# lizaibeim/mmla-audio

Measured on AMD Instinct MI355X. Metric: audio clips/sec (MFCC→logits) at 1/2/4/8 MI355X; MFCC max-abs-err vs librosa, higher is better.
Workload: dtype f16x3+f32

## Files before the change

### mmla_audio_amd/csrc/context.cpp

```cpp
#include <algorithm>
#include <cstdarg>
#include <cstdio>
#include <cstdlib>

#include "internal.h"

using namespace mmla;

namespace mmla __attribute__((visibility("hidden"))) {

int fail(mmla_ctx* c, int code, const char* fmt, ...) {
  char buf[512];
  va_list ap;
  va_start(ap, fmt);
  vsnprintf(buf, sizeof(buf), fmt, ap);
  va_end(ap);
  if (c) c->err = buf;
  return code;
}

static hipEvent_t prof_event(mmla_ctx* c) {
  if (!c->prof_pool.empty()) {
    hipEvent_t e = c->prof_pool.back();
    c->prof_pool.pop_back();
// ... 75 lines not shown
  }
  *out = c->ws[slot];
  return MMLA_OK;
}

int ws_release(mmla_ctx* c) {
  HIPCHK(c, hipStreamSynchronize(c->stream));
  for (size_t i = 0; i < c->ws.size(); ++i)
    if (c->ws[i]) {
      HIPCHK(c, hipFree(static_cast<char*>(c->ws[i]) - c->ws_guard[i]));
      c->ws[i] = nullptr;
      c->ws_size[i] = 0;
      c->ws_guard[i] = 0;
    }
  return MMLA_OK;
}

static int ws_check_guards(mmla_ctx* c) {
  std::vector<unsigned char> h(kGuardBytes);
  for (size_t slot = 0; slot < c->ws.size(); ++slot) {
    const size_t g = c->ws_guard[slot];
    if (!c->ws[slot] || !g) continue;
    for (int side = 0; side < 2; ++side) {
      const char* d = static_cast<const char*>(c->ws[slot]) + (side ? c->ws_size[slot] : -(ptrdiff_t)g);
      HIPCHK(c, hipMemcpy(h.data(), d, g, hipMemcpyDeviceToHost));
      for (size_t i = 0; i < g; ++i)
        if (h[i] != kGuardByte)
          return fail(c, MMLA_E_HIP, "workspace slot %zu: %s guard overwritten at byte %zu", slot,
                      side ? "trailing" : "leading", side ? i : g - i);
    }
  }
  return MMLA_OK;
}

int finish(mmla_ctx* c, bool dev) {
  HIPCHK(c, hipGetLastError());
  bool guarded = false;
  for (size_t g : c->ws_guard) guarded |= g != 0;
  if (!dev || guarded) HIPCHK(c, hipStreamSynchronize(c->stream));
  if (guarded) return ws_check_guards(c);
  return MMLA_OK;
}

constexpr double kOdBytesPerClip = 3.0 * 128 * 151 * 32 * 4 + 128 * 151 * 3 + 128 * 151 * 4 +
                                   19 * 128 * 4 + 512 * 4 + 64;
constexpr double kSiBytesPerClip = 4.0 * 256 * 32 * 4 + 256 * 39 * 4 + 8 * 128 * 4 + 512 * 4 +
                                   1024 * 4 + 64;

int64_t microbatch(mmla_ctx* c, bool od) {
  const int64_t user = od ? c->od_mb : c->si_mb;
  if (user > 0) return user;
  const int64_t cap = od ? c->od_mb_cap : c->si_mb_cap;
  size_t fr = 0, tot = 0;
  if (hipMemGetInfo(&fr, &tot) != hipSuccess) {
    (void)hipGetLastError();
    return cap;
  }
  double held = 0;
  for (size_t b : c->ws_size) held += (double)b;
  int64_t fit = (int64_t)(((double)fr + held) * 0.9 / (od ? kOdBytesPerClip : kSiBytesPerClip));
  fit = fit / kMinMicrobatch * kMinMicrobatch;
  return std::max(kMinMicrobatch, std::min(cap, fit));
}

}

struct EnvSwitch {
  const char* name;
  bool mmla_ctx::*no;
  int mmla_ctx::*num;
};
static const EnvSwitch kEnvSwitches[] = {
    {"MMLA_DEBUG_FAIL_ALLOC", nullptr, &mmla_ctx::debug_fail_allocs},
    {"MMLA_NO_SIU", &mmla_ctx::siu, nullptr},
    {"MMLA_NO_SIPU", &mmla_ctx::sipu, nullptr},
    {"MMLA_NO_SIFIN", &mmla_ctx::sifin, nullptr},
    {"MMLA_NO_SIPAIR", &mmla_ctx::sipair, nullptr},
    {"MMLA_NO_SICHAIN", &mmla_ctx::sichain, nullptr},
    {"MMLA_NO_LSTM_SPLIT", &mmla_ctx::lstm_split, nullptr},
    {"MMLA_LSTM_SPLIT_MAX", nullptr, &mmla_ctx::lstm_split_max},
    {"MMLA_DEBUG_LSTM_SPIN", nullptr, &mmla_ctx::lstm_spin},
    {"MMLA_NO_SIPAD", &mmla_ctx::si_pad_feat, nullptr},
    {"MMLA_NO_ODU", &mmla_ctx::odu, nullptr},
    {"MMLA_RB_TILE", &mmla_ctx::rbs, nullptr},
    {"MMLA_NO_PIN_OUT", &mmla_ctx::pin_small, nullptr},
};

extern "C" {

int mmla_abi_version(void) { return MMLA_ABI_VERSION; }

int mmla_create(int device, mmla_ctx** out) {
  if (!out) return MMLA_E_INVALID;
  *out = nullptr;
  int ndev = 0;
  if (hipGetDeviceCount(&ndev) != hipSuccess || ndev == 0) return MMLA_E_HIP;
  if (device < 0 || device >= ndev) return MMLA_E_INVALID;
  if (hipSetDevice(device) != hipSuccess) return MMLA_E_HIP;
  mmla_ctx* c = new mmla_ctx();
  c->device = device;
  for (const EnvSwitch& s : kEnvSwitches)
    if (const char* v = std::getenv(s.name)) {
      if (s.no) c->*s.no = std::atoi(v) == 0;
      else c->*s.num = std::atoi(v);
    }
  if (hipStreamCreateWithFlags(&c->own_stream, hipStreamDefault) != hipSuccess) {
    delete c;
    return MMLA_E_HIP;
  }
  c->stream = c->own_stream;
  if (hipMalloc(&c->range_dev, 4 * sizeof(int)) != hipSuccess ||
      hipMemset(c->range_dev, 0, 4 * sizeof(int)) != hipSuccess ||
      hipHostMalloc(&c->range_host, 2 * sizeof(int), hipHostMallocDefault) != hipSuccess) {
    mmla_destroy(c);
    return MMLA_E_HIP;
  }
  if (c->pin_small) {
    const unsigned fl = hipHostMallocMapped | hipHostMallocCoherent;
    if (hipHostMalloc(reinterpret_cast<void**>(&c->range_map), 64, fl) != hipSuccess ||
        hipHostGetDevicePointer(reinterpret_cast<void**>(&c->range_map_dev), c->range_map, 0) != hipSuccess ||
        hipHostMalloc(reinterpret_cast<void**>(&c->pin_out), kPinSlots * kPinSlotBytes, fl) != hipSuccess ||
        hipHostGetDevicePointer(reinterpret_cast<void**>(&c->pin_out_dev), c->pin_out, 0) != hipSuccess ||
        hipHostMalloc(reinterpret_cast<void**>(&c->pin_in), kPinInBytes, hipHostMallocDefault) != hipSuccess) {
      mmla_destroy(c);
      return MMLA_E_HIP;
    }
    c->range_map[0] = c->range_map[1] = 0;
  }
  OdFeTables ot;
  od_fe_build_tables(&ot);
  if (!od_fe_tables_ok(ot)) {
    mmla_destroy(c);
    return MMLA_E_INVALID;
  }
  SiFeTables st;
  si_fe_build_tables(&st);
  if (!si_fe_tables_ok(st)) {
    mmla_destroy(c);
    return MMLA_E_INVALID;
  }
  if (hipMalloc(&c->od_tables, sizeof(OdFeTables)) != hipSuccess ||
      hipMalloc(&c->si_tables, sizeof(SiFeTables)) != hipSuccess ||
      hipMemcpy(c->od_tables, &ot, sizeof(ot), hipMemcpyHostToDevice) != hipSuccess ||
      hipMemcpy(c->si_tables, &st, sizeof(st), hipMemcpyHostToDevice) != hipSuccess) {
    mmla_destroy(c);
    return MMLA_E_HIP;
  }
  *out = c;
  return MMLA_OK;
}

int mmla_destroy(mmla_ctx* c) {
  if (!c) return MMLA_E_INVALID;
  (void)hipSetDevice(c->device);
  if (c->stream) (void)hipStreamSynchronize(c->stream);
  free_allocs(c->od_allocs);
  free_allocs(c->si_allocs);
  for (size_t i = 0; i < c->ws.size(); ++i)
    if (c->ws[i]) (void)hipFree(static_cast<char*>(c->ws[i]) - c->ws_guard[i]);
  if (c->od_tables) (void)hipFree(c->od_tables);
  if (c->si_tables) (void)hipFree(c->si_tables);
  if (c->nr_tables) (void)hipFree(c->nr_tables);
  if (c->nr_thresh) (void)hipFree(c->nr_thresh);
  if (c->range_dev) (void)hipFree(c->range_dev);
  if (c->vad_state) (void)hipFree(c->vad_state);
  if (c->range_host) (void)hipHostFree(c->range_host);
// ... 121 lines not shown
```

### mmla_audio_amd/csrc/internal.h

```cpp
#pragma once
#include <hip/hip_runtime.h>

#include <cstdint>
#include <cstring>
#include <string>
#include <vector>

#include "../../include/mmla.h"
#include "nr.h"
#include "od_fe.h"
#include "si_fe.h"
#include "vad.h"

namespace mmla __attribute__((visibility("hidden"))) {

constexpr int OD_H = 128, OD_W = 151, OD_PIX = OD_H * OD_W;
constexpr int OD_IMG = OD_PIX * 3;
constexpr int SI_T = 256, SI_D = 39;
constexpr int SI_NEED_SAMPLES = 160 * 259 + 400;
constexpr int CH[9] = {32, 32, 32, 64, 64, 64, 128, 128, 128};
constexpr bool POOL[9] = {true, false, false, true, false, false, true, false, false};

struct ConvW {
  float* wt = nullptr;
// ... 5 lines not shown
  int kh = 0, kw = 0, cin = 0, cout = 0, cout_pad = 0, cin_pad = 0, kpad = 0;
  float wscale = 256.0f;
  float unscale() const { return 1.0f / (16.0f * wscale); }
};
struct BnW {
  float* scale = nullptr;
  float* shift = nullptr;
  int c = 0;
};
struct LstmW {
  float* wcat[2] = {nullptr, nullptr};
  float* bias[2] = {nullptr, nullptr};
  uint16_t* wth[2] = {nullptr, nullptr};
  uint16_t* wtl[2] = {nullptr, nullptr};
  float ws[2] = {256.0f, 256.0f};
};
struct ResUnitW {
  BnW bn_in, bn_mid;
  ConvW ca, cb, sc;
};
struct OdNet {
  ConvW stem;
  ResUnitW blk[9];
  LstmW lstm;
  float* head_w = nullptr;
  float* head_b = nullptr;
};
struct SiNet {
  ConvW stem;
  ResUnitW unit[9];
  BnW final_bn;
  LstmW lstm;
  ConvW dense;
  int k = 0, head = 0;
};

struct ProfRec {
  int stage;
  hipEvent_t a, b;
  double work;
};

constexpr int64_t kOdMicrobatch = 16384;
constexpr int64_t kSiMicrobatch = 65536;
constexpr int64_t kMinMicrobatch = 64;

constexpr size_t kPinSlotBytes = 64u << 10;
constexpr size_t kPinInBytes = 1u << 20;
constexpr int kPinSlots = 4;

}

struct mmla_ctx {
  bool prof_on = false;
  std::vector<mmla::ProfRec> prof_pending;
  std::vector<hipEvent_t> prof_pool;
  double prof_ms[MMLA_NSTAGES] = {0};
  double prof_work[MMLA_NSTAGES] = {0};
  int64_t prof_n[MMLA_NSTAGES] = {0};
  int device = 0;
  hipStream_t stream = nullptr;
  hipStream_t own_stream = nullptr;
  std::string err;
  OdFeTables* od_tables = nullptr;
  SiFeTables* si_tables = nullptr;
  bool od_loaded = false, si_loaded = false;
  mmla::OdNet od;
  mmla::SiNet si;
  std::vector<void*> od_allocs, si_allocs;
  std::vector<void*> ws;
  std::vector<size_t> ws_size;
  std::vector<size_t> ws_guard;
  int64_t od_mb = 0, si_mb = 0;
  int64_t od_mb_cap = mmla::kOdMicrobatch, si_mb_cap = mmla::kSiMicrobatch;
  int debug_fail_allocs = 0;
  int precision = MMLA_PREC_F16X3;
  bool siu = true;
  bool sipu = true;
  bool sifin = true;
  bool sipair = true;
  bool sichain = true;
  bool si_pad_feat = true;
  bool odu = true;
  bool rbs = true;
  bool lstm_split = true;
  int lstm_split_max = 128;
  int lstm_spin = 0;
  int* range_dev = nullptr;
  int* range_host = nullptr;
  bool pin_small = true;
  int* range_map = nullptr;
  int* range_map_dev = nullptr;
  char* pin_out = nullptr;
  char* pin_out_dev = nullptr;
  char* pin_in = nullptr;
  int* range_ptr = nullptr;
  int* timeout_ptr = nullptr;
  int64_t lstm_split_reruns = 0;
  int64_t range_reruns = 0;
  bool od_f32_only = false, si_f32_only = false;
  bool loading_f16_bad = false;
  VadState* vad_state = nullptr;
  int64_t vad_streams = 0;
  NrTables* nr_tables = nullptr;
  float* nr_thresh = nullptr;
  bool nr_ready = false;
};

namespace mmla __attribute__((visibility("hidden"))) {

int fail(mmla_ctx* c, int code, const char* fmt, ...);

#define HIPCHK(ctx, expr)                                                                        \
  do {                                                                                           \
    hipError_t e_ = (expr);                                                                      \
    if (e_ != hipSuccess)                                                                        \
      return mmla::fail(ctx, MMLA_E_HIP, "%s failed: %s (%s:%d)", #expr, hipGetErrorString(e_), \
                        __FILE__, __LINE__);                                                     \
  } while (0)

#define CHK(expr)              \
  do {                         \
    int r_ = (expr);           \
    if (r_ != MMLA_OK) return r_; \
  } while (0)

int prof_begin(mmla_ctx* c, int stage);
void prof_end(mmla_ctx* c, int idx, double work);
int prof_collect(mmla_ctx* c);

#define LAUNCH(c, st, wk, expr)                  \
  do {                                           \
    const int pi_ = mmla::prof_begin((c), (st)); \
    HIPCHK((c), (expr));                         \
    mmla::prof_end((c), pi_, (wk));              \
  } while (0)

enum Slot {
  S_PCM = 0, S_LENS, S_IMG, S_X, S_T1, S_T2, S_T3, S_SEQ, S_HOUT, S_LOGIT, S_FEAT, S_SILENT,
  S_OUT0, S_OUT1, S_OUT2, S_OUT3, S_IN,
  S_NR_S, S_NR_BITS, S_NR_FMAX, S_NR_FRAMES, S_NR_ITEMS, S_NR_Y, S_NR_ROWS,
  S_VAD_SPEECH, S_VAD_OUT, S_VAD_LENS, S_RS_TR, S_RS_WIN, S_LSTM,
  S_TRAIN
};

int ws_get(mmla_ctx* c, int slot, size_t bytes, void** out);
int ws_release(mmla_ctx* c);
int64_t microbatch(mmla_ctx* c, bool od);
int finish(mmla_ctx* c, bool dev);
void free_allocs(std::vector<void*>& al);

template <typename T>
int in_ptr(mmla_ctx* c, const T* user, size_t count, bool dev, int slot, const T** d) {
  *d = user;
  if (dev || !user) return MMLA_OK;
  void* p = nullptr;
  CHK(ws_get(c, slot, count * sizeof(T), &p));
  HIPCHK(c, hipMemcpyAsync(p, user, count * sizeof(T), hipMemcpyHostToDevice, c->stream));
  *d = static_cast<const T*>(p);
  return MMLA_OK;
}

template <typename T>
int out_ptr(mmla_ctx* c, T* user, int64_t off, size_t count, bool dev, int slot, T** d) {
  if (!user) {
    *d = nullptr;
// ... 45 lines not shown
```

### mmla_audio_amd/csrc/net_runners.cpp

```cpp
#include <algorithm>

#include "conv.h"
#include "conv_h3.h"
#include "internal.h"
#include "nets.h"
#include "odu.h"
#include "resblk.h"
#include "siu.h"

using namespace mmla;

namespace {

ConvArgs conv_args(const ConvW& w, const float* x, float* y, int n, int h, int wd, int stride,
                   const BnW* bn, int pro, int epi, const float* res) {
  ConvArgs a{};
  a.x = x;
  a.wt = w.wt;
  a.bias = w.bias;
  a.scale = bn ? bn->scale : nullptr;
  a.shift = bn ? bn->shift : nullptr;
  a.res = res;
  a.y = y;
  a.n = n;
  a.h = h;
  a.w = wd;
  a.cin = w.cin;
  a.ho = (h + stride - 1) / stride;
  a.wo = (wd + stride - 1) / stride;
  a.cout = w.cout;
  a.cout_pad = w.cout_pad;
  a.ldy = w.cout;
  a.kh = w.kh;
  a.kw = w.kw;
  a.stride = stride;
  const int th = std::max((a.ho - 1) * stride + w.kh - h, 0);
  const int tw = std::max((a.wo - 1) * stride + w.kw - wd, 0);
  a.pad_h = th / 2;
  a.pad_w = tw / 2;
  a.pro = pro;
  a.epi = epi;
  return a;
}

double conv_flops(const ConvArgs& a) {
  return 2.0 * (double)a.n * a.ho * a.wo * a.kh * a.kw * a.cin * a.cout;
}

int conv_run(mmla_ctx* c, const ConvArgs& a, int stage = MMLA_STAGE_CONV) {
  LAUNCH(c, stage, conv_flops(a), conv_launch(a, c->stream));
  return MMLA_OK;
}

ConvH3Args conv_h3_args(const ConvW& w, const float* x, float* y, int n, int h, int wd, const BnW* bn,
                        int pro, int epi, const float* res, int* range_flag) {
  ConvH3Args a{};
  a.x = x;
  a.wh = w.wh;
  a.wl = w.wl;
  a.unscale = w.unscale();
  a.bias = w.bias;
  a.scale = bn ? bn->scale : nullptr;
  a.shift = bn ? bn->shift : nullptr;
  a.res = res;
  a.y = y;
  a.n = n;
  a.h = h;
  a.w = wd;
  a.cin = w.cin;
  a.cin_pad = w.cin_pad;
  a.cout = w.cout;
  a.cout_pad = w.cout_pad;
  a.kh = w.kh;
  a.kw = w.kw;
  a.pad_h = (w.kh - 1) / 2;
  a.pad_w = (w.kw - 1) / 2;
  a.pro = pro;
  a.epi = epi;
  a.range_flag = range_flag;
  return a;
}

int conv_spatial(mmla_ctx* c, const ConvW& w, const float* x, float* y, int n, int h, int wd,
                 const BnW* bn, int pro, int epi, const float* res, bool pool_out = false,
                 int pool_in_h = 0, const ConvW* sc = nullptr, const float* sc_x = nullptr,
                 int sc_h = 0) {
  if (c->precision == MMLA_PREC_F16X3 && w.wh) {
    ConvH3Args a = conv_h3_args(w, x, y, n, h, wd, bn, pro, epi, res, c->range_ptr);
    double sc_flops = 0.0;
    if (sc && sc_x) {
      a.sc_x = sc_x;
      a.sc_wh = sc->wh;
      a.sc_wl = sc->wl;
      a.sc_bias = sc->bias;
      a.sc_cin = sc->cin;
      a.sc_h = sc_h;
      a.sc_unscale = sc->unscale();
      sc_flops = sc_h > 0 ? 2.0 * n * h * sc->cin * sc->cout
                          : 2.0 * n * ((h + 1) / 2) * ((wd + 1) / 2) * sc->cin * sc->cout;
    }
    a.pool_in = pool_in_h > 0;
    a.h_in = pool_in_h;
    a.pool_out = pool_out ? 1 : 0;
    LAUNCH(c, MMLA_STAGE_CONV, 2.0 * n * h * wd * w.kh * w.kw * w.cin * w.cout + sc_flops,
           conv_h3_launch(a, c->stream));
    return MMLA_OK;
  }
  ConvArgs a = conv_args(w, x, y, n, h, wd, 1, bn, pro, epi, res);
  if (!pool_out) return conv_run(c, a);
  return fail(c, MMLA_E_INVALID, "pooled epilogue needs the 3xFP16 conv path");
}

int ws_floats(mmla_ctx* c, int slot, size_t count, float** out) {
  void* p = nullptr;
  CHK(ws_get(c, slot, count * sizeof(float), &p));
  *out = static_cast<float*>(p);
  return MMLA_OK;
}

double lstm_flops(int64_t n, int T, int D) { return 2.0 * n * T * 2 * (256.0 + D) * 1024.0; }

hipError_t lstm_run(mmla_ctx* c, const LstmW& L, const float* seq, int64_t n, int T, float* out) {
  if (c->precision == MMLA_PREC_F16X3 && L.wth[0] && c->lstm_split &&
      n <= std::min(c->lstm_split_max, bilstm_h3_split_max_clips())) {
    void* ws = nullptr;
    if (ws_get(c, S_LSTM, bilstm_h3_split_ws_bytes(), &ws) != MMLA_OK) return hipErrorOutOfMemory;
    return bilstm_h3_split_launch(seq, (int)n, T, 128, L.wth[0], L.wtl[0], L.wth[1], L.wtl[1],
                                  L.bias[0], L.bias[1], out, c->range_ptr, L.ws[0], L.ws[1], ws,
                                  c->timeout_ptr, c->lstm_spin, c->stream);
  }
  if (c->precision == MMLA_PREC_F16X3 && L.wth[0])
    return bilstm_h3_launch(seq, (int)n, T, 128, L.wth[0], L.wtl[0], L.wth[1], L.wtl[1], L.bias[0],
                            L.bias[1], out, c->range_ptr, L.ws[0], L.ws[1], c->stream);
  return bilstm_launch(seq, (int)n, T, 128, L.wcat[0], L.wcat[1], L.bias[0], L.bias[1], out,
                       c->stream);
}


enum OdPath {
  OD_STRIPS,
  OD_TILES,
  OD_ODU,
  OD_PAIR
};
struct OdChoice {
  OdPath path;
  bool stem;
};

bool strips_ok(const ResUnitW& B, bool pool, int h, int w) {
  return B.ca.wh && B.cb.wh && (!pool || B.sc.wh) && B.ca.cin_pad == B.ca.cin && B.ca.cout_pad == 32 &&
         B.cb.cin_pad == 32 && B.cb.cout_pad == 32 && B.cb.kh == 4 && B.cb.kw == 1 &&
         (!pool || (B.sc.cin_pad == B.ca.cin && B.sc.cout_pad == 32)) &&
         rbs_supported(h, w, B.ca.cin, B.ca.cout, pool);
}

bool tiles_ok(const ResUnitW& B, bool pool) {
  return B.ca.fh && B.cb.fh && B.cb.kpad == 4 * B.cb.cin && (!pool || B.sc.fh) &&
         resblk_supported(B.ca.cin, B.ca.cout, pool);
}

bool odu_ok(const ResUnitW& B, bool pool, int h, int w) {
  return B.ca.wh && B.cb.wh && (!pool || B.sc.wh) && odu_supported(h, w, B.ca.cin, B.ca.cout, pool) &&
         B.ca.cin_pad == B.ca.cin && B.ca.cout_pad == B.ca.cout && B.cb.cin == B.ca.cout &&
         B.cb.cout == B.ca.cout && B.cb.cin_pad == B.cb.cin && B.cb.cout_pad == B.cb.cout &&
         B.cb.kh == 4 && B.cb.kw == 1 &&
         (!pool || (B.sc.cin == B.ca.cin && B.sc.cout == B.ca.cout && B.sc.cout_pad == B.sc.cout));
}

OdChoice od_choose(const mmla_ctx* c, const ResUnitW& B, int b, int h, int w, int stop) {
  OdChoice k{OD_PAIR, false};
  if (c->precision != MMLA_PREC_F16X3) return k;
  if (c->rbs && strips_ok(B, POOL[b], h, w)) k.path = OD_STRIPS;
  else if (tiles_ok(B, POOL[b])) k.path = OD_TILES;
  else if (c->odu && odu_ok(B, POOL[b], h, w)) k.path = OD_ODU;
  k.stem = b == 0 && stop != 0 && (k.path == OD_STRIPS || k.path == OD_TILES);
  return k;
}

ResBlkArgs resblk_args(const ResUnitW& B, bool pool, bool fused, const float* x, float* y, int64_t n,
                       int h, int w, int* range_flag, const ConvW* stem, const uint8_t* img_u8,
                       const float* img_f32) {
  ResBlkArgs r{};
  r.x = x;
  r.y = y;
  r.w1h = fused ? B.ca.fh : B.ca.wh;
  r.w1l = fused ? B.ca.fl : B.ca.wl;
  r.b1 = B.ca.bias;
  r.u1 = B.ca.unscale();
  r.s1 = B.bn_in.scale;
  r.t1 = B.bn_in.shift;
  r.w2h = fused ? B.cb.fh : B.cb.wh;
  r.w2l = fused ? B.cb.fl : B.cb.wl;
  r.b2 = B.cb.bias;
  r.u2 = B.cb.unscale();
  r.s2 = B.bn_mid.scale;
  r.t2 = B.bn_mid.shift;
  if (pool) {
    r.wsh = fused ? B.sc.fh : B.sc.wh;
    r.wsl = fused ? B.sc.fl : B.sc.wl;
    r.bs = B.sc.bias;
    r.us = B.sc.unscale();
  }
  if (stem) {
    r.x = nullptr;
    r.img8 = img_u8;
    r.imgf = img_u8 ? nullptr : img_f32;
    r.wst = stem->wt;
    r.bst = stem->bias;
    r.ldst = stem->cout_pad;
  }
  r.n = (int)n;
  r.h = h;
  r.w = w;
  r.range_flag = range_flag;
  return r;
}

OduArgs odu_args(const ResUnitW& B, bool pool, const float* x, float* y, int64_t n, int* range_flag) {
  OduArgs o{};
  o.x = x;
  o.y = y;
  o.wah = B.ca.wh;
  o.wal = B.ca.wl;
  o.wbh = B.cb.wh;
  o.wbl = B.cb.wl;
  o.ba = B.ca.bias;
  o.bb = B.cb.bias;
  o.s_in = B.bn_in.scale;
  o.t_in = B.bn_in.shift;
  o.s_mid = B.bn_mid.scale;
  o.t_mid = B.bn_mid.shift;
  o.ua = B.ca.unscale();
  o.ub = B.cb.unscale();
  o.n = (int)n;
  o.range_flag = range_flag;
  if (pool) {
    o.wsh = B.sc.wh;
    o.wsl = B.sc.wl;
    o.bs = B.sc.bias;
    o.us = B.sc.unscale();
  }
  return o;
}

double od_block_flops(const ResUnitW& B, bool pool, int64_t n, int h, int w) {
  return 2.0 * n * h * w * (9.0 * B.ca.cin * B.ca.cout + 4.0 * B.cb.cin * B.cb.cout) +
         (pool ? 2.0 * n * ((h + 1) / 2) * ((w + 1) / 2) * B.sc.cin * B.sc.cout : 0.0);
}

int od_block_pair(mmla_ctx* c, const ResUnitW& B, bool pool, int n, int h, int w, float* X, float*& T1,
                  float*& T2, float** out) {
  CHK(conv_spatial(c, B.ca, X, T1, n, h, w, &B.bn_in, PRO_BN_ELU, EPI_BIAS, nullptr));
  if (!pool) {
    *out = X;
    return conv_spatial(c, B.cb, T1, X, n, h, w, &B.bn_mid, PRO_BN_ELU, EPI_ADD, X);
  }
  if (c->precision != MMLA_PREC_F16X3) {
    CHK(conv_spatial(c, B.cb, T1, T2, n, h, w, &B.bn_mid, PRO_BN_ELU, EPI_BIAS, nullptr));
    ConvArgs s = conv_args(B.sc, X, T1, n, h, w, 2, nullptr, PRO_NONE, EPI_ADD_POOL, T2);
    s.hp = h;
    s.wp = w;
    CHK(conv_run(c, s));
  } else if (B.sc.wh && B.sc.cout == B.cb.cout && B.cb.cout_pad == B.sc.cout_pad) {
    CHK(conv_spatial(c, B.cb, T1, T2, n, h, w, &B.bn_mid, PRO_BN_ELU, EPI_BIAS, nullptr, true, 0, &B.sc,
                     X));
    std::swap(T1, T2);
  } else {
    CHK(conv_spatial(c, B.cb, T1, T2, n, h, w, &B.bn_mid, PRO_BN_ELU, EPI_BIAS, nullptr, true));
    CHK(conv_run(c, conv_args(B.sc, X, T1, n, h, w, 2, nullptr, PRO_NONE, EPI_ADD, T2)));
  }
  *out = T1;
  return MMLA_OK;
}

}

namespace mmla __attribute__((visibility("hidden"))) {

int run_od_net(mmla_ctx* c, const uint8_t* img_u8, const float* img_f32, int64_t n, float* probs,
               int32_t* argmax, OdGate gate, int stop, const float** tap, int64_t* tap_n) {
  const OdNet& W = c->od;
  const size_t big = (size_t)n * OD_PIX * 32;
  float *X, *T1, *T2, *SEQ, *H;
  CHK(ws_floats(c, S_X, big, &X));
  CHK(ws_floats(c, S_T1, big, &T1));
  CHK(ws_floats(c, S_T2, big, &T2));
  CHK(ws_floats(c, S_SEQ, (size_t)n * 19 * 128, &SEQ));
  CHK(ws_floats(c, S_HOUT, (size_t)n * 512, &H));
  const double stem_flops = 2.0 * n * OD_PIX * 3 * 16;
  const OdChoice first = od_choose(c, W.blk[0], 0, OD_H, OD_W, stop);
  if (!first.stem)
    LAUNCH(c, MMLA_STAGE_GLUE, stem_flops,
           od_stem_launch(img_u8, img_f32, n * OD_PIX, W.stem.cout_pad, W.stem.wt, W.stem.bias, X,
                          c->stream));
  int h = OD_H, w = OD_W;
  if (stop == 0) {
    *tap = X;
    *tap_n = n * OD_PIX * 16;
    return MMLA_OK;
  }
  for (int b = 0; b < 9; ++b) {
    const ResUnitW& B = W.blk[b];
    const bool pool = POOL[b];
    const OdChoice k = b == 0 ? first : od_choose(c, B, b, h, w, stop);
    const double flops = od_block_flops(B, pool, n, h, w) + (k.stem ? stem_flops : 0.0);
    float* out = T1;
    switch (k.path) {
      case OD_STRIPS:
      case OD_TILES: {
        const bool tiles = k.path == OD_TILES;
        const ResBlkArgs r = resblk_args(B, pool, tiles, X, T1, n, h, w, c->range_ptr,
                                         k.stem ? &W.stem : nullptr, img_u8, img_f32);
        LAUNCH(c, MMLA_STAGE_CONV, flops,
               tiles ? resblk_launch(r, B.ca.cin, B.ca.cout, pool, c->stream)
                     : rbs_launch(r, B.ca.cin, B.ca.cout, pool, c->stream));
        break;
      }
      case OD_ODU:
        LAUNCH(c, MMLA_STAGE_CONV, flops,
               odu_launch(odu_args(B, pool, X, T1, n, c->range_ptr), h, w, B.ca.cin, B.ca.cout, pool,
                          c->stream));
        break;
      case OD_PAIR:
        CHK(od_block_pair(c, B, pool, (int)n, h, w, X, T1, T2, &out));
        break;
    }
    if (pool) {
      h = (h + 1) / 2;
      w = (w + 1) / 2;
    }
    if (out != X) std::swap(X, T1);
    if (stop == b + 1) {
      *tap = X;
      *tap_n = n * h * w * CH[b];
      return MMLA_OK;
    }
  }
  LAUNCH(c, MMLA_STAGE_GLUE, (double)n * h * w * 128,
         mean_h_launch(X, (int)n, h, w, 128, SEQ, c->stream));
  if (stop == 10) {
    *tap = SEQ;
    *tap_n = n * w * 128;
    return MMLA_OK;
  }
  LAUNCH(c, MMLA_STAGE_LSTM, lstm_flops(n, w, 128),
         lstm_run(c, W.lstm, SEQ, n, w, H));
  if (stop == 11) {
    *tap = H;
    *tap_n = n * 512;
    return MMLA_OK;
  }
  LAUNCH(c, MMLA_STAGE_HEAD, 2.0 * n * 512 * 2,
         od_head_launch(H, (int)n, W.head_w, W.head_b, probs, argmax,
                        gate.lens, gate.clip_len, gate.silent, c->stream));
  return MMLA_OK;
}

}


namespace {

bool siu_ok(const ResUnitW& U, int cin) {
  return U.ca.wh && U.cb.wh && siu_supported(cin) && U.ca.cin == cin && U.ca.cout == cin && U.cb.cin == cin &&
         U.cb.cout == cin && U.ca.cin_pad == cin && U.ca.cout_pad == cin && U.cb.cout_pad == cin;
}

bool sipu_ok(const ResUnitW& U, int cin) {
  return U.ca.wh && U.cb.wh && U.sc.wh && sipu_supported(cin, U.ca.cout) && U.ca.cin_pad == cin &&
         U.ca.cout_pad == U.ca.cout && U.cb.cin == U.ca.cout && U.cb.cout == U.ca.cout &&
         U.cb.cout_pad == U.ca.cout && U.sc.cin == cin && U.sc.cout == U.ca.cout &&
         U.sc.cout_pad == U.ca.cout;
}

SiuArgs siu_args(const ResUnitW& U, const float* x, float* y, int64_t n, int t, int* range_flag,
                 int t_src = 0) {
  SiuArgs s{};
  s.n = (int)n;
  s.t = t;
  s.range_flag = range_flag;
  s.x = x;
  s.y = y;
  s.wah = U.ca.wh;
  s.wal = U.ca.wl;
  s.wbh = U.cb.wh;
  s.wbl = U.cb.wl;
  s.ba = U.ca.bias;
  s.bb = U.cb.bias;
  s.s_in = U.bn_in.scale;
  s.t_in = U.bn_in.shift;
  s.s_mid = U.bn_mid.scale;
  s.t_mid = U.bn_mid.shift;
  s.ua = U.ca.unscale();
  s.ub = U.cb.unscale();
  if (t_src > 0) {
    s.t_src = t_src;
    s.wsh = U.sc.wh;
    s.wsl = U.sc.wl;
    s.bs = U.sc.bias;
    s.us = U.sc.unscale();
  }
  return s;
}

}
// ... 118 lines not shown
```

Before: 170,300.

## Add two-strip fused residual-block kernel for late OD blocks

Adds a new fused residual-unit kernel (odw) for the 128-channel OD blocks at 32x38 (pooled) and 16x19. Each workgroup handles two column strips, so every weight fragment loaded from global memory feeds MFMAs for both strips. It also prefetches the next tap's weights and the next LDS A-fragment, pinned with sched_group_barrier to overlap loads with the f16x3 MFMAs. The kernel is chosen by default over the odu path for these shapes, at the cost of more LDS and registers per block and one more specialised code path to keep correct.

Measured after the change: 172,200, median of 6. 1.01x the previous value.

```diff
diff --git a/mmla_audio_amd/csrc/context.cpp b/mmla_audio_amd/csrc/context.cpp
--- a/mmla_audio_amd/csrc/context.cpp
+++ b/mmla_audio_amd/csrc/context.cpp
@@ -181,6 +181,7 @@
     {"MMLA_DEBUG_LSTM_SPIN", nullptr, &mmla_ctx::lstm_spin},
     {"MMLA_NO_SIPAD", &mmla_ctx::si_pad_feat, nullptr},
     {"MMLA_NO_ODU", &mmla_ctx::odu, nullptr},
+    {"MMLA_NO_ODW", &mmla_ctx::odw, nullptr},
     {"MMLA_RB_TILE", &mmla_ctx::rbs, nullptr},
     {"MMLA_NO_PIN_OUT", &mmla_ctx::pin_small, nullptr},
 };
diff --git a/mmla_audio_amd/csrc/internal.h b/mmla_audio_amd/csrc/internal.h
--- a/mmla_audio_amd/csrc/internal.h
+++ b/mmla_audio_amd/csrc/internal.h
@@ -111,6 +111,7 @@
   bool sichain = true;
   bool si_pad_feat = true;
   bool odu = true;
+  bool odw = true;
   bool rbs = true;
   bool lstm_split = true;
   int lstm_split_max = 128;
diff --git a/mmla_audio_amd/csrc/net_runners.cpp b/mmla_audio_amd/csrc/net_runners.cpp
--- a/mmla_audio_amd/csrc/net_runners.cpp
+++ b/mmla_audio_amd/csrc/net_runners.cpp
@@ -5,6 +5,7 @@
 #include "internal.h"
 #include "nets.h"
 #include "odu.h"
+#include "odw.h"
 #include "resblk.h"
 #include "siu.h"
 
@@ -141,6 +142,7 @@
   OD_STRIPS,
   OD_TILES,
   OD_ODU,
+  OD_ODW,
   OD_PAIR
 };
 struct OdChoice {
@@ -168,12 +170,16 @@
          (!pool || (B.sc.cin == B.ca.cin && B.sc.cout == B.ca.cout && B.sc.cout_pad == B.sc.cout));
 }
 
+bool odw_ok(const ResUnitW& B, bool pool, int h, int w) {
+  return odw_supported(h, w, B.ca.cin, B.ca.cout, pool);
+}
+
 OdChoice od_choose(const mmla_ctx* c, const ResUnitW& B, int b, int h, int w, int stop) {
   OdChoice k{OD_PAIR, false};
   if (c->precision != MMLA_PREC_F16X3) return k;
   if (c->rbs && strips_ok(B, POOL[b], h, w)) k.path = OD_STRIPS;
   else if (tiles_ok(B, POOL[b])) k.path = OD_TILES;
-  else if (c->odu && odu_ok(B, POOL[b], h, w)) k.path = OD_ODU;
+  else if (c->odu && odu_ok(B, POOL[b], h, w)) k.path = c->odw && odw_ok(B, POOL[b], h, w) ? OD_ODW : OD_ODU;
   k.stem = b == 0 && stop != 0 && (k.path == OD_STRIPS || k.path == OD_TILES);
   return k;
 }
@@ -318,10 +324,13 @@
         break;
       }
       case OD_ODU:
+      case OD_ODW: {
+        const OduArgs o = odu_args(B, pool, X, T1, n, c->range_ptr);
         LAUNCH(c, MMLA_STAGE_CONV, flops,
-               odu_launch(odu_args(B, pool, X, T1, n, c->range_ptr), h, w, B.ca.cin, B.ca.cout, pool,
-                          c->stream));
+               k.path == OD_ODW ? odw_launch(o, h, w, B.ca.cin, B.ca.cout, pool, c->stream)
+                                : odu_launch(o, h, w, B.ca.cin, B.ca.cout, pool, c->stream));
         break;
+      }
       case OD_PAIR:
         CHK(od_block_pair(c, B, pool, (int)n, h, w, X, T1, T2, &out));
         break;
diff --git a/mmla_audio_amd/csrc/odw.h b/mmla_audio_amd/csrc/odw.h
--- /dev/null
+++ b/mmla_audio_amd/csrc/odw.h
@@ -0,0 +1,5 @@
+#pragma once
+#include "odu.h"
+
+bool odw_supported(int h, int w, int cin, int c, bool pool);
+hipError_t odw_launch(const OduArgs& a, int h, int w, int cin, int c, bool pool, hipStream_t stream);
diff --git a/mmla_audio_amd/csrc/odw.hip b/mmla_audio_amd/csrc/odw.hip
--- /dev/null
+++ b/mmla_audio_amd/csrc/odw.hip
@@ -0,0 +1,463 @@
+#include "common.h"
+#include "conv.h"
+#include "odw.h"
+
+namespace {
+
+typedef float f32x16 __attribute__((ext_vector_type(16)));
+typedef _Float16 f16x8 __attribute__((ext_vector_type(8)));
+typedef _Float16 f16x4 __attribute__((ext_vector_type(4)));
+
+constexpr int CK = 32;
+constexpr int KS = CK / 16;
+constexpr int NS = 2;
+constexpr float ACT_SCALE = 16.0f;
+constexpr float SPLIT_MAX = 65504.0f;
+
+MMLA_DEV __amdgpu_buffer_rsrc_t odw_rsrc(const void* p) {
+  const uint64_t u = reinterpret_cast<uint64_t>(p);
+  const uint32_t lo = __builtin_amdgcn_readfirstlane((uint32_t)u);
+  const uint32_t hi = __builtin_amdgcn_readfirstlane((uint32_t)(u >> 32));
+  return __builtin_amdgcn_make_buffer_rsrc(reinterpret_cast<void*>(((uint64_t)hi << 32) | lo), (short)0,
+                                           (int)0x7fffffff, 0x00020000);
+}
+MMLA_DEV f16x8 odw_frag(__amdgpu_buffer_rsrc_t r, size_t uoff, int lofs) {
+  return __builtin_bit_cast(f16x8, __builtin_amdgcn_raw_buffer_load_b128(r, (uint32_t)lofs * 2u, (int)(uoff * 2), 0));
+}
+
+MMLA_DEV float bn_elu16(float v, float sc16, float sh16) { return elu16(fmaf(v, sc16, sh16)); }
+MMLA_DEV float4 x16(float4 v) { return make_float4(ACT_SCALE * v.x, ACT_SCALE * v.y, ACT_SCALE * v.z, ACT_SCALE * v.w); }
+
+MMLA_DEV void split4(float4 v, f16x4& h, f16x4& l) {
+  h[0] = (_Float16)v.x;
+  h[1] = (_Float16)v.y;
+  h[2] = (_Float16)v.z;
+  h[3] = (_Float16)v.w;
+  const uint2 hu = __builtin_bit_cast(uint2, h);
+  l = __builtin_bit_cast(f16x4, make_uint2(split_lo2(v.x, v.y, hu.x), split_lo2(v.z, v.w, hu.y)));
+}
+
+MMLA_DEV float amax4(float r, float4 v) {
+  return fmaxf(r, fmaxf(fmaxf(fabsf(v.x), fabsf(v.y)), fmaxf(fabsf(v.z), fabsf(v.w))));
+}
+
+template <int LA, int NR>
+MMLA_DEV void odw_pin_group() {
+  if constexpr (LA > 0) {
+    if constexpr (NR > 0) __builtin_amdgcn_sched_group_barrier(0x100, NR, 0);
+    __builtin_amdgcn_sched_group_barrier(0x008, 3, 0);
+    __builtin_amdgcn_sched_barrier(0);
+  }
+}
+
+template <int H, int W, int CIN, int C, int TW, bool POOL, bool DBUF, int LA, int LB>
+__global__ void __launch_bounds__(256, 2) odw_kernel(OduArgs a) {
+  constexpr int NW = 4, NT = 64 * NW;
+  constexpr int NB = LA + 1;
+  constexpr int WN = C / 32, WM = NW / WN;
+  constexpr int M = H * TW;
+  constexpr int MT = M / (WM * 32);
+  constexpr int NTL = NS * MT;
+  static_assert(MT * WM * 32 == M && WN * WM == NW, "tiling");
+  static_assert(!POOL || (TW == 2 && H % 2 == 0 && W % 2 == 0 && MT <= 4), "pool strips");
+  static_assert(POOL || CIN == C, "residual blocks keep their width");
+  constexpr int TLW = (W + TW - 1) / TW;
+  constexpr int XP = TW + 2, XH = H + 2, NXP = XH * XP;
+  constexpr int LDX = TW == 2 ? CK : CK + 8;
+  constexpr int XRP = TW == 2 ? 144 : TW == 4 ? 288 : XP * LDX;
+  constexpr bool XSW = TW == 2;
+  constexpr int LDT = C + 8;
+  constexpr int T1S = (H + 2) * TW * LDT;
+  constexpr int T1TOT = (NS * (H + 2) + 1) * TW * LDT;
+  constexpr int NCHX = CIN / CK, NCH = C / CK;
+  constexpr bool DB = DBUF && NCHX > 1;
+  constexpr int XBUF = XH * XRP;
+  constexpr int XTOT = DB ? 2 * XBUF : XBUF;
+  constexpr int PLANE = NS * XTOT > T1TOT ? NS * XTOT : T1TOT;
+  constexpr int QPP = CK / 4;
+  constexpr int MAXT = (NXP * QPP + NT - 1) / NT;
+  static_assert(NT % QPP == 0, "a thread's channel quad is fixed");
+  __shared__ __attribute__((aligned(16))) _Float16 lhi[PLANE];
+  __shared__ __attribute__((aligned(16))) _Float16 llo[PLANE];
+
+  const int tid = threadIdx.x, lane = tid & 63, wave = tid >> 6;
+  const int wm = wave / WN, wn = wave - (wave / WN) * WN;
+  const uint32_t bid = xcd_block_id();
+  const int64_t strips = (int64_t)a.n * TLW;
+  bool live[NS];
+  int64_t clip[NS];
+  int w0[NS];
+  __amdgpu_buffer_rsrc_t rxc[NS];
+#pragma unroll
+  for (int sp = 0; sp < NS; ++sp) {
+    const int64_t sid = (int64_t)bid * NS + sp;
+    live[sp] = sid < strips;
+    clip[sp] = live[sp] ? sid / TLW : 0;
+    w0[sp] = live[sp] ? (int)(sid - clip[sp] * TLW) * TW : W + TW;
+    rxc[sp] = __builtin_amdgcn_make_buffer_rsrc(const_cast<float*>(a.x + clip[sp] * ((int64_t)H * W * CIN)), (short)0,
+                                                live[sp] ? (int)(H * W * CIN * 4) : 0, 0x00020000);
+  }
+  const int koff = (lane >> 5) * 8;
+  const int hsel = 4 * (lane >> 5);
+  const int cob = wn * 32;
+  const int lofs = wn * 512 + lane * 8;
+  constexpr size_t kstr = (size_t)(C / 32) * 512;
+  float rmax = 0.0f;
+
+  int mpix[MT];
+#pragma unroll
+  for (int mt = 0; mt < MT; ++mt) mpix[mt] = (wm * MT + mt) * 32 + (lane & 31);
+
+  f32x16 acc[NTL];
+#pragma unroll
+  for (int t = 0; t < NTL; ++t)
+#pragma unroll
+    for (int i = 0; i < 16; ++i) acc[t][i] = 0.0f;
+
+  {
+    const __amdgpu_buffer_rsrc_t rh = odw_rsrc(a.wah), rl = odw_rsrc(a.wal);
+    constexpr size_t tap_stride = (size_t)C * CIN;
+    const int q = tid % QPP;
+    const int kx0 = XSW ? 8 * ((lane >> 5) ^ (lane & 1)) : koff;
+    const int kx1 = XSW ? 8 * ((lane >> 5) ^ (lane & 1) ^ 1) : koff;
+    auto load_stage = [&](int sp, int ch, int buf) {
+      const int ci = ch * CK + 4 * q;
+      const float4 sc = x16(*reinterpret_cast<const float4*>(a.s_in + ci));
+      const float4 sh = x16(*reinterpret_cast<const float4*>(a.t_in + ci));
+      float4 pre[MAXT];
+      uint32_t valid = 0;
+#pragma unroll
+      for (int j = 0; j < MAXT; ++j) {
+        const int task = tid + j * NT;
+        const int px = task / QPP;
+        const int ih = px / XP - 1, iw = w0[sp] + px % XP - 1;
+        const bool ok = task < NXP * QPP && ih >= 0 && ih < H && iw >= 0 && iw < W;
+        pre[j] = __builtin_bit_cast(float4, __builtin_amdgcn_raw_buffer_load_b128(
+                                                rxc[sp], ok ? (uint32_t)((ih * W + iw) * CIN + ci) * 4u : 0x80000000u, 0, 0));
+        valid |= (uint32_t)ok << j;
+      }
+      asm volatile("" : "+v"(valid));
+      _Float16* const xh = lhi + sp * XTOT + buf * XBUF;
+      _Float16* const xl = llo + sp * XTOT + buf * XBUF;
+#pragma unroll
+      for (int j = 0; j < MAXT; ++j) {
+        const int task = tid + j * NT;
+        if (task >= NXP * QPP) continue;
+        float4 v = pre[j];
+        if (valid & (1u << j)) {
+          v.x = bn_elu16(v.x, sc.x, sh.x);
+          v.y = bn_elu16(v.y, sc.y, sh.y);
+          v.z = bn_elu16(v.z, sc.z, sh.z);
+          v.w = bn_elu16(v.w, sc.w, sh.w);
+        }
+        rmax = amax4(rmax, v);
+        f16x4 hv, lv;
+        split4(v, hv, lv);
+        const int px = task / QPP;
+        const int cx = px % XP;
+        const int xo = (px / XP) * XRP + cx * LDX + (XSW ? 8 * ((q >> 1) ^ (cx & 1)) + 4 * (q & 1) : 4 * q);
+        *reinterpret_cast<f16x4*>(xh + xo) = hv;
+        *reinterpret_cast<f16x4*>(xl + xo) = lv;
+      }
+    };
+    if constexpr (DB) {
+#pragma unroll
+      for (int sp = 0; sp < NS; ++sp) load_stage(sp, 0, 0);
+      __syncthreads();
+    }
+#pragma unroll 1
+    for (int ch = 0; ch < NCHX; ++ch) {
+      const int buf = DB ? (ch & 1) : 0;
+      f16x8 bh[KS], bl[KS];
+#pragma unroll
+      for (int s = 0; s < KS; ++s) {
+        bh[s] = odw_frag(rh, (size_t)(ch * KS + s) * kstr, lofs);
+        bl[s] = odw_frag(rl, (size_t)(ch * KS + s) * kstr, lofs);
+      }
+      if constexpr (!DB) {
+        if (ch > 0) __syncthreads();
+#pragma unroll
+        for (int sp = 0; sp < NS; ++sp) load_stage(sp, ch, 0);
+        __syncthreads();
+      }
+      constexpr int NG = 9 * KS * NTL;
+      auto aoff = [&](int g) {
+        const int t = g % NTL, s = (g / NTL) % KS, tap = g / (NTL * KS);
+        const int dy = tap / 3, dx = tap - (tap / 3) * 3;
+        const int m = mpix[t % MT];
+        return (t / MT) * XTOT + buf * XBUF + (m / TW + dy) * XRP + (m % TW + dx) * LDX + 16 * s + (dx & 1 ? kx1 : kx0);
+      };
+      f16x8 fah[NB], fal[NB];
+#pragma unroll
+      for (int d = 0; d < LA; ++d) {
+        fah[d] = *reinterpret_cast<const f16x8*>(lhi + aoff(d));
+        fal[d] = *reinterpret_cast<const f16x8*>(llo + aoff(d));
+      }
+#pragma unroll
+      for (int tap = 0; tap < 9; ++tap) {
+        f16x8 nbh[KS], nbl[KS];
+        if (tap + 1 < 9) {
+#pragma unroll
+          for (int s = 0; s < KS; ++s) {
+            const size_t u = (tap + 1) * tap_stride + (size_t)(ch * KS + s) * kstr;
+            nbh[s] = odw_frag(rh, u, lofs);
+            nbl[s] = odw_frag(rl, u, lofs);
+          }
+        }
+#pragma unroll
+        for (int s = 0; s < KS; ++s)
+#pragma unroll
+          for (int t = 0; t < NTL; ++t) {
+            const int g = (tap * KS + s) * NTL + t;
+            if (g + LA < NG) {
+              fah[(g + LA) % NB] = *reinterpret_cast<const f16x8*>(lhi + aoff(g + LA));
+              fal[(g + LA) % NB] = *reinterpret_cast<const f16x8*>(llo + aoff(g + LA));
+            }
+            const f16x8 ah = fah[g % NB], al = fal[g % NB];
+            acc[t] = __builtin_amdgcn_mfma_f32_32x32x16_f16(bl[s], ah, acc[t], 0, 0, 0);
+            acc[t] = __builtin_amdgcn_mfma_f32_32x32x16_f16(bh[s], al, acc[t], 0, 0, 0);
+            acc[t] = __builtin_amdgcn_mfma_f32_32x32x16_f16(bh[s], ah, acc[t], 0, 0, 0);
+            if (g + LA < NG) odw_pin_group<LA, 2>(); else odw_pin_group<LA, 0>();
+          }
+        if (tap + 1 < 9) {
+#pragma unroll
+          for (int s = 0; s < KS; ++s) {
+            bh[s] = nbh[s];
+            bl[s] = nbl[s];
+          }
+        }
+      }
+      if constexpr (DB) {
+        if (ch + 1 < NCHX) {
+#pragma unroll
+          for (int sp = 0; sp < NS; ++sp) load_stage(sp, ch + 1, buf ^ 1);
+          __syncthreads();
+        }
+      }
+    }
+  }
+  __syncthreads();
+
+#pragma unroll
+  for (int qd = 0; qd < 4; ++qd) {
+    const int c0 = cob + 8 * qd + hsel;
+    const float4 b4 = *reinterpret_cast<const float4*>(a.ba + c0);
+    const float4 s4 = x16(*reinterpret_cast<const float4*>(a.s_mid + c0));
+    const float4 t4 = x16(*reinterpret_cast<const float4*>(a.t_mid + c0));
+#pragma unroll
+    for (int t = 0; t < NTL; ++t) {
+      const int sp = t / MT;
+      const int m = mpix[t % MT];
+      const int i = m / TW, c = m % TW;
+      float4 v = make_float4(0.f, 0.f, 0.f, 0.f);
+      if (w0[sp] + c < W) {
+        v.x = bn_elu16(fmaf(acc[t][4 * qd + 0], a.ua, b4.x), s4.x, t4.x);
+        v.y = bn_elu16(fmaf(acc[t][4 * qd + 1], a.ua, b4.y), s4.y, t4.y);
+        v.z = bn_elu16(fmaf(acc[t][4 * qd + 2], a.ua, b4.z), s4.z, t4.z);
+        v.w = bn_elu16(fmaf(acc[t][4 * qd + 3], a.ua, b4.w), s4.w, t4.w);
+      }
+      rmax = amax4(rmax, v);
+      f16x4 hv, lv;
+      split4(v, hv, lv);
+      const int px = (i + 1) * TW + c;
+      *reinterpret_cast<f16x4*>(lhi + sp * T1S + px * LDT + c0) = hv;
+      *reinterpret_cast<f16x4*>(llo + sp * T1S + px * LDT + c0) = lv;
+    }
+  }
+  for (int e = tid; e < (2 * NS + 1) * TW * (LDT / 8); e += NT) {
+    const int z = e / (LDT / 8), k8 = e - z * (LDT / 8);
+    const int zr = z / TW;
+    const int row = zr == 0 ? 0 : ((zr + 1) / 2) * (H + 2) - 1 + ((zr + 1) & 1);
+    const int px = row * TW + (z - zr * TW);
+    *reinterpret_cast<f16x8*>(lhi + px * LDT + 8 * k8) = f16x8{};
+    *reinterpret_cast<f16x8*>(llo + px * LDT + 8 * k8) = f16x8{};
+  }
+
+  float4 rsd[POOL ? 1 : NS][POOL ? 1 : MT][4];
+  auto load_rsd = [&](int sp) {
+#pragma unroll
+    for (int mt = 0; mt < MT; ++mt) {
+      const int m = mpix[mt];
+      const int i = m / TW, c = m % TW;
+      const bool ok = w0[sp] + c < W;
+#pragma unroll
+      for (int qd = 0; qd < 4; ++qd)
+        rsd[sp][mt][qd] = __builtin_bit_cast(float4, __builtin_amdgcn_raw_buffer_load_b128(
+                              rxc[sp], ok ? (uint32_t)((i * W + w0[sp] + c) * C + cob + 8 * qd + hsel) * 4u : 0x80000000u, 0, 0));
+    }
+  };
+  if constexpr (!POOL) load_rsd(0);
+#pragma unroll
+  for (int t = 0; t < NTL; ++t)
+#pragma unroll
+    for (int i = 0; i < 16; ++i) acc[t][i] = 0.0f;
+  __syncthreads();
+
+  {
+    const __amdgpu_buffer_rsrc_t rh = odw_rsrc(a.wbh), rl = odw_rsrc(a.wbl);
+    constexpr size_t tap_stride = (size_t)C * C;
+#pragma unroll 1
+    for (int ch = 0; ch < NCH; ++ch) {
+      f16x8 bh[KS], bl[KS];
+#pragma unroll
+      for (int s = 0; s < KS; ++s) {
+        bh[s] = odw_frag(rh, (size_t)(ch * KS + s) * kstr, lofs);
+        bl[s] = odw_frag(rl, (size_t)(ch * KS + s) * kstr, lofs);
+      }
+      constexpr int NG = 4 * KS * NTL;
+      auto boff = [&](int g) {
+        const int t = g % NTL, s = (g / NTL) % KS, tap = g / (NTL * KS);
+        const int m = mpix[t % MT];
+        return (t / MT) * T1S + ((m / TW + tap) * TW + m % TW) * LDT + ch * CK + 16 * s + koff;
+      };
+      f16x8 fah[LB + 1], fal[LB + 1];
+#pragma unroll
+      for (int d = 0; d < LB; ++d) {
+        fah[d] = *reinterpret_cast<const f16x8*>(lhi + boff(d));
+        fal[d] = *reinterpret_cast<const f16x8*>(llo + boff(d));
+      }
+#pragma unroll
+      for (int tap = 0; tap < 4; ++tap) {
+        f16x8 nbh[KS], nbl[KS];
+        if (tap + 1 < 4) {
+#pragma unroll
+          for (int s = 0; s < KS; ++s) {
+            const size_t u = (tap + 1) * tap_stride + (size_t)(ch * KS + s) * kstr;
+            nbh[s] = odw_frag(rh, u, lofs);
+            nbl[s] = odw_frag(rl, u, lofs);
+          }
+        }
+#pragma unroll
+        for (int s = 0; s < KS; ++s)
+#pragma unroll
+          for (int t = 0; t < NTL; ++t) {
+            const int g = (tap * KS + s) * NTL + t;
+            if (g + LB < NG) {
+              fah[(g + LB) % (LB + 1)] = *reinterpret_cast<const f16x8*>(lhi + boff(g + LB));
+              fal[(g + LB) % (LB + 1)] = *reinterpret_cast<const f16x8*>(llo + boff(g + LB));
+            }
+            const f16x8 ah = fah[g % (LB + 1)], al = fal[g % (LB + 1)];
+            if constexpr (POOL) {
+              acc[t] = __builtin_amdgcn_mfma_f32_32x32x16_f16(ah, bl[s], acc[t], 0, 0, 0);
+              acc[t] = __builtin_amdgcn_mfma_f32_32x32x16_f16(al, bh[s], acc[t], 0, 0, 0);
+              acc[t] = __builtin_amdgcn_mfma_f32_32x32x16_f16(ah, bh[s], acc[t], 0, 0, 0);
+            } else {
+              acc[t] = __builtin_amdgcn_mfma_f32_32x32x16_f16(bl[s], ah, acc[t], 0, 0, 0);
+              acc[t] = __builtin_amdgcn_mfma_f32_32x32x16_f16(bh[s], al, acc[t], 0, 0, 0);
+              acc[t] = __builtin_amdgcn_mfma_f32_32x32x16_f16(bh[s], ah, acc[t], 0, 0, 0);
+            }
+            if (g + LB < NG) odw_pin_group<LB, 2>(); else odw_pin_group<LB, 0>();
+          }
+        if (tap + 1 < 4) {
+#pragma unroll
+          for (int s = 0; s < KS; ++s) {
+            bh[s] = nbh[s];
+            bl[s] = nbl[s];
+          }
+        }
+      }
+    }
+  }
+
+  if constexpr (!POOL) {
+    load_rsd(1);
+#pragma unroll
+    for (int t = 0; t < NTL; ++t) {
+      const int sp = t / MT;
+      const int m = mpix[t % MT];
+      const int i = m / TW, c = m % TW;
+      if (w0[sp] + c >= W) continue;
+#pragma unroll
+      for (int qd = 0; qd < 4; ++qd) {
+        const int c0 = cob + 8 * qd + hsel;
+        const float4 b4 = *reinterpret_cast<const float4*>(a.bb + c0);
+        const float4 r = rsd[sp][t % MT][qd];
+        float4 v = make_float4(fmaf(acc[t][4 * qd + 0], a.ub, b4.x), fmaf(acc[t][4 * qd + 1], a.ub, b4.y),
+                               fmaf(acc[t][4 * qd + 2], a.ub, b4.z), fmaf(acc[t][4 * qd + 3], a.ub, b4.w));
+        v = make_float4(v.x + r.x, v.y + r.y, v.z + r.z, v.w + r.w);
+        *reinterpret_cast<float4*>(a.y + ((clip[sp] * H + i) * W + w0[sp] + c) * C + c0) = v;
+      }
+    }
+  } else {
+    f32x16 sacc[NS];
+#pragma unroll
+    for (int sp = 0; sp < NS; ++sp)
+#pragma unroll
+      for (int i = 0; i < 16; ++i) sacc[sp][i] = 0.0f;
+    {
+      const int rho = lane & 31;
+      const int smt = rho >> 3, sq = rho & 3, sh = (rho >> 2) & 1;
+      const int m0 = (wm * MT + (smt < MT ? smt : 0)) * 32 + 8 * sq + 4 * sh;
+      const __amdgpu_buffer_rsrc_t rh = odw_rsrc(a.wsh), rl = odw_rsrc(a.wsl);
+#pragma unroll
+      for (int s = 0; s < CIN / 16; ++s) {
+        const f16x8 wh = odw_frag(rh, (size_t)s * kstr, lofs);
+        const f16x8 wl = odw_frag(rl, (size_t)s * kstr, lofs);
+#pragma unroll
+        for (int sp = 0; sp < NS; ++sp) {
+          const bool sok = smt < MT && live[sp];
+          const float* sx = a.x + ((clip[sp] * H + m0 / TW) * W + (live[sp] ? w0[sp] : 0)) * CIN + koff;
+          float4 x0 = make_float4(0.f, 0.f, 0.f, 0.f), x1 = x0;
+          if (sok) {
+            x0 = *reinterpret_cast<const float4*>(sx + 16 * s);
+            x1 = *reinterpret_cast<const float4*>(sx + 16 * s + 4);
+          }
+          x0 = x16(x0);
+          x1 = x16(x1);
+          rmax = amax4(amax4(rmax, x0), x1);
+          f16x4 h0, l0, h1, l1;
+          split4(x0, h0, l0);
+          split4(x1, h1, l1);
+          const f16x8 xh = {h0[0], h0[1], h0[2], h0[3], h1[0], h1[1], h1[2], h1[3]};
+          const f16x8 xl = {l0[0], l0[1], l0[2], l0[3], l1[0], l1[1], l1[2], l1[3]};
+          sacc[sp] = __builtin_amdgcn_mfma_f32_32x32x16_f16(xh, wl, sacc[sp], 0, 0, 0);
+          sacc[sp] = __builtin_amdgcn_mfma_f32_32x32x16_f16(xl, wh, sacc[sp], 0, 0, 0);
+          sacc[sp] = __builtin_amdgcn_mfma_f32_32x32x16_f16(xh, wh, sacc[sp], 0, 0, 0);
+        }
+      }
+    }
+    const int co = cob + (lane & 31);
+    const float b = a.bb[co], bsc = a.bs[co];
+#pragma unroll
+    for (int t = 0; t < NTL; ++t) {
+      const int sp = t / MT, mt = t % MT;
+      if (!live[sp]) continue;
+#pragma unroll
+      for (int qd = 0; qd < 4; ++qd) {
+        const int m0 = (wm * MT + mt) * 32 + 8 * qd + hsel;
+        const int i0 = m0 / TW;
+        float mx = fmaf(acc[t][4 * qd], a.ub, b);
+        mx = fmaxf(mx, fmaf(acc[t][4 * qd + 1], a.ub, b));
+        mx = fmaxf(mx, fmaf(acc[t][4 * qd + 2], a.ub, b));
+        mx = fmaxf(mx, fmaf(acc[t][4 * qd + 3], a.ub, b));
+        mx += fmaf(sacc[sp][4 * mt + qd], a.us, bsc);
+        a.y[((clip[sp] * (H / 2) + i0 / 2) * (W / 2) + w0[sp] / 2) * C + co] = mx;
+      }
+    }
+  }
+  if (!(rmax < SPLIT_MAX) && a.range_flag) *a.range_flag = 1;
+}
+
+template <int H, int W, int CIN, int C, int TW, bool POOL, bool DBUF, int LA, int LB>
+hipError_t launch(const OduArgs& a, hipStream_t s) {
+  constexpr int TLW = (W + TW - 1) / TW;
+  const int64_t blocks = ((int64_t)a.n * TLW + NS - 1) / NS;
+  hipLaunchKernelGGL((odw_kernel<H, W, CIN, C, TW, POOL, DBUF, LA, LB>), dim3((unsigned)blocks), dim3(256), 0, s, a);
+  return hipGetLastError();
+}
+
+}
+
+bool odw_supported(int h, int w, int cin, int c, bool pool) {
+  return (h == 32 && w == 38 && cin == 64 && c == 128 && pool) ||
+         (h == 16 && w == 19 && cin == 128 && c == 128 && !pool);
+}
+
+hipError_t odw_launch(const OduArgs& a, int h, int w, int cin, int c, bool pool, hipStream_t s) {
+  if (a.n == 0) return hipSuccess;
+  if (!a.x || !a.y || a.x == a.y || !odw_supported(h, w, cin, c, pool) ||
+      (pool && (!a.wsh || !a.wsl || !a.bs)))
+    return hipErrorInvalidValue;
+  if (pool) return launch<32, 38, 64, 128, 2, true, true, 1, 1>(a, s);
+  return launch<16, 19, 128, 128, 4, false, false, 1, 1>(a, s);
+}
```
